# stevenabreu7/SparseRNNs

Measured on AMD Instinct MI355X. Metric: frames/sec at w8a16 S5 dim_scale=0.5 (NDNS shape), bit-exact vs CPU fxprun, higher is better.
Workload: dtype int32

## Files before the change

sparsernns_amd/csrc/proj_p.hpp:

```cpp
#pragma once
#ifdef S5_PHASE_PROF
__device__ long long g_phase_prof[2048 * 8];
#define PHASE_DECL unsigned prof_last, prof_a0 = 0, prof_a1 = 0, prof_a2 = 0, prof_a3 = 0, prof_a4 = 0, prof_a5 = 0, prof_a6 = 0, prof_a7 = 0; \
    { unsigned long long t_; asm volatile("s_memtime %0\n\ts_waitcnt lgkmcnt(0)" : "=s"(t_)); prof_last = __builtin_amdgcn_readfirstlane((unsigned)t_); }
#define PHASE_MARK(i, reg) do { unsigned long long t_; asm volatile("v_cmp_eq_u32 vcc, %1, %1\n\ts_nop 0\n\ts_memtime %0\n\ts_waitcnt lgkmcnt(0)" : "=s"(t_) : "v"(reg) : "memory", "vcc"); \
    const unsigned tl_ = __builtin_amdgcn_readfirstlane((unsigned)t_); prof_a##i = __builtin_amdgcn_readfirstlane(prof_a##i + (tl_ - prof_last)); prof_last = tl_; } while (0)
#define PHASE_DUMP do { if (threadIdx.x == 0 && blockIdx.x < 2048) { long long *o_ = g_phase_prof + blockIdx.x * 8; o_[0] = prof_a0; o_[1] = prof_a1; o_[2] = prof_a2; o_[3] = prof_a3; \
    o_[4] = prof_a4; o_[5] = prof_a5; o_[6] = prof_a6; o_[7] = prof_a7; } } while (0)
#else
#define PHASE_DECL
#define PHASE_MARK(i, reg)
#define PHASE_DUMP
#endif
#include "mfma_bn.hpp"

namespace s5 {

__host__ __device__ constexpr int shape_channels(int NT) { return (NT == 2 || NT == 5) ? 32 * NT - 16 : 32 * NT; }

template <int HC, int HP, int KP>
__device__ __forceinline__ void zero_plane_tail(int8_t *base, int rows)
{
    if constexpr (HC != HP) {
        static_assert(HP - HC == 16, "half a tile");
        for (int i = threadIdx.x; i < rows; i += blockDim.x) *reinterpret_cast<v4i *>(base + i * KP + HC) = v4i{0, 0, 0, 0};
    }
}

__device__ __forceinline__ void planes8_from_i32(const int32_t (&v)[8], v2i &hi, v2i &lo)
{
#pragma unroll
    for (int j = 0; j < 2; ++j) {
        const unsigned p01 = perm((unsigned)v[4 * j + 1], (unsigned)v[4 * j], 0x05010400u);
        const unsigned p23 = perm((unsigned)v[4 * j + 3], (unsigned)v[4 * j + 2], 0x05010400u);
        lo[j] = (int)(perm(p23, p01, 0x05040100u) ^ 0x80808080u);
        hi[j] = (int)perm(p23, p01, 0x07060302u);
    }
}

struct StepRange {
    int32_t t_lo, t_len;
};
template <int FT = 64>
__device__ __forceinline__ void tile_of(int64_t tile, const StepRange &sr, int64_t &b, int &t, int &nvalid)
{
    const int tps = (sr.t_len + FT - 1) / FT;
    b = tile / tps;
    const int tt = (int)(tile - b * tps) * FT;
    t = sr.t_lo + tt;
    nvalid = sr.t_len - tt < FT ? sr.t_len - tt : FT;
}

template <int FT = 64>
struct TileWalk {
    int tps, db, dti;
    int b, ti;
    __device__ __forceinline__ TileWalk(int64_t tile0, const StepRange &sr, unsigned step)
    {
        tps = (sr.t_len + FT - 1) / FT;
        db = (int)(step / (unsigned)tps); dti = (int)(step % (unsigned)tps);
        b = (int)((unsigned)tile0 / (unsigned)tps); ti = (int)((unsigned)tile0 % (unsigned)tps);
    }
    __device__ __forceinline__ void advance()
    {
        b += db; ti += dti;
        if (ti >= tps) { ti -= tps; ++b; }
    }
    __device__ __forceinline__ TileWalk next() const { TileWalk n = *this; n.advance(); return n; }
    __device__ __forceinline__ int t(const StepRange &sr) const { return sr.t_lo + ti * FT; }
    __device__ __forceinline__ int nvalid(const StepRange &sr) const { const int left = sr.t_len - ti * FT; return left < FT ? left : FT; }
};

template <int KS, int NT, bool TRACE, int SM = 0, int NC = NT>
__global__ __launch_bounds__(64 * NT, TRACE ? 2 : KS == 5 ? 3 : 4) void k_bproj_p(BprojM2Args a, GroupOff go)
{
    {
        const int64_t g = blockIdx.y;
        gshift(a.bn.dyn, g * go.ws); gshift(a.bn.xe.dyn, g * go.ws); gshift(a.x, g * go.ws); gshift(a.bq, g * go.ws); gshift(a.u, g * go.ws);
        gshift(a.ext, g * go.ws); gshift(a.status, g * go.status); gshift(a.status_exps, g * go.status);
    }
    static_assert(NC == NT || 2 * NC == NT || 4 * NC == NT, "column tiles per workgroup");
    constexpr int H = shape_channels(KS), HP = 32 * KS, FT = 64, KP = 32 * KS + 16, PC = 16 * NC, SUB0_STEP = NT / NC;
    constexpr int VPF = H / 8;
    constexpr int NTHR = 64 * NT;
    constexpr int NV = FT * VPF / NTHR;
    constexpr int NCT = 1;
    constexpr int PLANE = FT * KP;
    static_assert(FT * VPF % NTHR == 0, "tile shape");
    extern __shared__ __attribute__((aligned(16))) int8_t smem[];
    int32_t *tab = reinterpret_cast<int32_t *>(smem);
    int8_t *Xh = smem + 16 * HP, *Xl = Xh + 2 * PLANE;
    zero_plane_tail<H, HP, KP>(Xh, 4 * FT);
    const int l = threadIdx.x & 63, r = l & 31, h = l >> 5, wave = threadIdx.x >> 6;
    const int wct = wave % NC, wsub = wave / NC;
    const StepRange sr{a.t_lo, a.t_len};
    const int64_t tiles = (a.N / a.L) * ((sr.t_len + FT - 1) / FT);
    int64_t tile = blockIdx.x;

    v4i raw[NV];
    auto fetch = [&](const TileWalk<FT> &tw) {
        const int64_t b = tw.b;
        const int t = tw.t(sr), nv = tw.nvalid(sr);
        const char *xb = reinterpret_cast<const char *>(a.x + (b * a.L + t) * H);
#pragma unroll
        for (int i = 0; i < NV; ++i) {
            const int v = threadIdx.x + NTHR * i;
            int f = v / VPF;
            f = f < nv ? f : nv - 1;
            raw[i] = *reinterpret_cast<const v4i *>(xb + 2u * (unsigned)(f * H + 8 * (v % VPF)));
        }
    };
    TileWalk<FT> walk(tile, sr, gridDim.x);
    if (tile < tiles) fetch(walk);
    v4i wreg[NCT][KS];
    int32_t csv[NCT];
#pragma unroll
    for (int c = 0; c < NCT; ++c) {
        const int col = 32 * (wct + NC * c) + r;
        csv[c] = a.w.cs128[col];
#pragma unroll
        for (int ks = 0; ks < KS; ++ks)
            wreg[c][ks] = *reinterpret_cast<const v4i *>(a.w.wt + (size_t)col * a.w.Kp + 32 * ks + 16 * h);
    }
    const LayerDyn d = a.ext ? bn_finalize_mm_body(a.bn, a.ext, H, const_cast<LayerDyn *>(a.bn.dyn), a.status, a.status_exps, a.bn.xe.get(), a.ext_reps,
                                                   blockIdx.x == 0)
                             : *a.bn.dyn;
    const Bn16 bn = bn16_setup(a.bn, d, tab, H);
    constexpr bool LAZY = KS == 3 && !TRACE;
    ResolveU16 rz{};
    int lazy_arm = 0;
    if constexpr (LAZY) {
        if (a.lazy) {
            gshift_nn(a.lazy, (int64_t)blockIdx.y * go.ws);
            rz = resolve_u16_setup(a.lazy->res.post);
            lazy_arm = 1 + rz.arm;
        }
    }
    __syncthreads();

    prologue_loads_done();
    for (int it = 0; tile < tiles; tile += gridDim.x, ++it, walk.advance()) {
        const int64_t b0 = walk.b;
        const int t0 = walk.t(sr), nvalid = walk.nvalid(sr);
        const int64_t n0 = b0 * a.L + t0;
        char *ub = reinterpret_cast<char *>(a.u + n0 * H);
        int8_t *xh = Xh + (it & 1) * PLANE, *xl = Xl + (it & 1) * PLANE;
#pragma unroll
        for (int i = 0; i < NV; ++i) {
            const int v = threadIdx.x + NTHR * i, f = v / VPF, og = v % VPF;
            const int64_t n = n0 + f;
            int32_t xin[8], t[8], u[8];
            if constexpr (LAZY) {
                if (lazy_arm == 1 + RES_RIGHT) {
#pragma unroll
                    for (int e = 0; e < 4; ++e) raw[i][e] = (int)resolve_u16_pair<RES_RIGHT>(rz, (uint32_t)raw[i][e]);
                } else if (lazy_arm) {
#pragma unroll
                    for (int e = 0; e < 4; ++e) raw[i][e] = (int)resolve_u16_pair<RES_GENERIC>(rz, (uint32_t)raw[i][e]);
                }
            }
            unpack8_i16(raw[i], xin);
            bn16_x4(bn, reinterpret_cast<const int32_t(&)[4]>(xin[0]), 8 * og, reinterpret_cast<int32_t(&)[4]>(t[0]),
                    reinterpret_cast<int32_t(&)[4]>(u[0]));
            bn16_x4(bn, reinterpret_cast<const int32_t(&)[4]>(xin[4]), 8 * og + 4, reinterpret_cast<int32_t(&)[4]>(t[4]),
                    reinterpret_cast<int32_t(&)[4]>(u[4]));
            if (f < nvalid && (TRACE || !a.no_u)) {
                const v2i p0 = pack4_i16(u[0], u[1], u[2], u[3]), p1 = pack4_i16(u[4], u[5], u[6], u[7]);
                *reinterpret_cast<v4i *>(ub + 2u * (unsigned)(f * H + 8 * og)) = v4i{p0[0], p0[1], p1[0], p1[1]};
                if (TRACE) {
#pragma unroll
                    for (int e = 0; e < 8; ++e) {
                        if (a.tr_pre_s5) a.tr_pre_s5[n * H + 8 * og + e] = t[e];
                        if (a.tr_u) a.tr_u[n * H + 8 * og + e] = u[e];
                    }
                }
            }
            v2i hi, lo;
            planes8_from_i32(u, hi, lo);
            *reinterpret_cast<v2i *>(xh + f * KP + 8 * og) = hi;
            *reinterpret_cast<v2i *>(xl + f * KP + 8 * og) = lo;
        }
        if (tile + gridDim.x < tiles) fetch(walk.next());
        __syncthreads();
#pragma unroll
        for (int c = 0; c < NCT; ++c) {
            const int col = 32 * (wct + NC * c) + r;
            const int cc = SM >= 2 ? (r >> 4) : (col >= PC ? 1 : 0), p = SM >= 2 ? 16 * (wct + NC * c) + (r & 15) : col - cc * PC;
            const int rs = cc ? a.rs_im : a.rs_re, bits = cc ? a.bim_bits : a.bre_bits, sh = cc ? a.sh_im : a.sh_re;
            const int lsh = sh < 0 ? -sh : 0, rsh = sh > 0 ? sh : 0;
            SatB sbu;
            sbu.hi = (int32_t)((1u << (bits - 1)) - 1u); sbu.lo = ~sbu.hi;
            asm volatile("" : "+v"(sbu.lo), "+v"(sbu.hi));
#pragma unroll
            for (int sub0 = 0; sub0 < 2; sub0 += SUB0_STEP) {
                const int sub = sub0 + wsub;
                if (SUB0_STEP > 2 && sub >= 2) break;
                const int8_t *rowh = xh + (32 * sub + r) * KP + 16 * h, *rowl = xl + (32 * sub + r) * KP + 16 * h;
                v16i acc;
#pragma unroll
                for (int i = 0; i < 16; ++i) acc[i] = 0;
#pragma unroll
                for (int ks = 0; ks < KS; ++ks)
                    acc = __builtin_amdgcn_mfma_i32_32x32x32_i8(*reinterpret_cast<const v4i *>(rowh + 32 * ks), wreg[c][ks], acc, 0, 0, 0);
#pragma unroll
                for (int i = 0; i < 16; ++i) acc[i] = wadd(wshl(acc[i], 8), csv[c]);
#pragma unroll
                for (int ks = 0; ks < KS; ++ks)
                    acc = __builtin_amdgcn_mfma_i32_32x32x32_i8(*reinterpret_cast<const v4i *>(rowl + 32 * ks), wreg[c][ks], acc, 0, 0, 0);
#pragma unroll
                for (int g = 0; g < 4; ++g) {
                    const int o = 32 * sub + 8 * g + 4 * h;
                    const bool live = o < nvalid;
                    {
                        v4i q;
#pragma unroll
                        for (int e = 0; e < 4; ++e) {
                            const int32_t bu = sat(asr(acc[4 * g + e], rs), sbu);
                            q[e] = asr(wshl(bu, lsh), rsh);
                            if (TRACE && o + e < nvalid) {
                                if (!cc && a.tr_bu_re) a.tr_bu_re[(n0 + o + e) * PC + p] = bu;
                                if (cc && a.tr_bu_im) a.tr_bu_im[(n0 + o + e) * PC + p] = bu;
                            }
                        }
                        if (SM == 3) {
                            const int32_t o0 = __builtin_amdgcn_ds_swizzle(q[0], 0x401f), o2 = __builtin_amdgcn_ds_swizzle(q[2], 0x401f);
                            const v2i item = pack4_i16(o0, o2, q[1], q[3]);
                            if (live && (a.live_slots <= 0 || p < a.live_slots)) {
                                char *qb = reinterpret_cast<char *>(reinterpret_cast<int16_t *>(a.bq) + pair16_half(b0, t0 >> 2, 0, 0, a.TB, PC));
                                const unsigned qo = 2u * (unsigned)((((((p >> 5) * (a.TB >> 1) + (o >> 3)) << 6) + 2 * (p & 31) + cc) * 8) + 4 * ((o >> 2) & 1));
                                *reinterpret_cast<v2i *>(qb + qo) = item;
                            }
                        } else if (SM == 2) {
                            const int32_t kc = cc ? 0 : a.k_re;
                            const int32_t k0 = wadd(wshl(q[0], 16), kc), k2 = wadd(wshl(q[2], 16), kc);
                            v4i item;
                            item[0] = __builtin_amdgcn_ds_swizzle(k0, 0x401f);
                            item[1] = __builtin_amdgcn_ds_swizzle(k2, 0x401f);
                            item[2] = wadd(wshl(q[1], 16), kc);
                            item[3] = wadd(wshl(q[3], 16), kc);
                            if (live) *reinterpret_cast<v4i *>(a.bq + pair_word(b0, (t0 + o) >> 2, p, a.TB, PC) + 4 * cc) = item;
                        } else if (SM == 1) {
                            if (live && (a.live_slots <= 0 || p < a.live_slots))
                                *reinterpret_cast<v2i *>(reinterpret_cast<int16_t *>(a.bq) + native_word(b0, t0 + o, p, cc, a.TB, PC)) =
                                    pack4_i16(q[0], q[1], q[2], q[3]);
                        } else if (live)
                            *reinterpret_cast<v4i *>(a.bq + native_word(b0, t0 + o, p, cc, a.TB, PC)) = q;
                    }
                }
            }
        }
    }
}

using v2u16 = __attribute__((ext_vector_type(2))) unsigned short;

struct CfgOp {
    int l, r, b;
    SatB sb;
    __device__ __forceinline__ int32_t operator()(int32_t d) const { return sat(asr(wshl(d, l), r), sb); }
};
__device__ __forceinline__ CfgOp make_cfg(bool on, int bits, int e, int bits2, int e2)
{
    CfgOp c;
    c.l = on && e2 > e ? e2 - e : 0;
    c.r = on && e > e2 ? e - e2 : 0;
    const int b1 = on && e2 != e ? bits : 32, b2 = on && bits > bits2 ? bits2 : 32;
    c.b = b1 < b2 ? b1 : b2;
    c.sb = sat_bounds(c.b);
    return c;
}

template <int KSTEPS>
__device__ __forceinline__ void mfma_planes(v16i &acc, const v4i (&w)[KSTEPS], const int8_t *rowh, const int8_t *rowl,
                                            const int32_t *cs)
{
#pragma unroll
    for (int i = 0; i < 16; ++i) acc[i] = 0;
#pragma unroll
    for (int ks = 0; ks < KSTEPS; ++ks)
        acc = __builtin_amdgcn_mfma_i32_32x32x32_i8(w[ks], *reinterpret_cast<const v4i *>(rowh + 32 * ks), acc, 0, 0, 0);
#pragma unroll
    for (int g = 0; g < 4; ++g) {
        const v4i c = *reinterpret_cast<const v4i *>(cs + 8 * g);
#pragma unroll
        for (int e = 0; e < 4; ++e) acc[4 * g + e] = wadd(wshl(acc[4 * g + e], 8), c[e]);
    }
#pragma unroll
    for (int ks = 0; ks < KSTEPS; ++ks)
        acc = __builtin_amdgcn_mfma_i32_32x32x32_i8(w[ks], *reinterpret_cast<const v4i *>(rowl + 32 * ks), acc, 0, 0, 0);
}

template <int KSTEPS, int NPL>
__device__ __forceinline__ void mfma_nplanes(v16i &acc, const v4i (&w)[KSTEPS], const int8_t *row0, int plane_stride,
                                             const int32_t *cs)
{
#pragma unroll
    for (int i = 0; i < 16; ++i) acc[i] = 0;
#pragma unroll
    for (int pl = NPL - 1; pl >= 0; --pl) {
        if (pl != NPL - 1) {
#pragma unroll
            for (int g = 0; g < 4; ++g) {
                const v4i c = *reinterpret_cast<const v4i *>(cs + 8 * g);
#pragma unroll
                for (int e = 0; e < 4; ++e) acc[4 * g + e] = wadd(wshl(acc[4 * g + e], 8), c[e]);
            }
        }
#pragma unroll
        for (int ks = 0; ks < KSTEPS; ++ks) {
            acc = __builtin_amdgcn_mfma_i32_32x32x32_i8(w[ks], *reinterpret_cast<const v4i *>(row0 + pl * plane_stride + 32 * ks), acc, 0, 0, 0);
        }
    }
}

enum { IO_I32 = 0, IO_F32 = 1, IO_I16 = 2 };

template <int NT>
__global__ __launch_bounds__(384, 3) void k_enc_p(EncArgs a, float *ext, int ext_reps, GroupOff go)
{
    constexpr int IO = IO_I32;
#include "proj_enc_body.inc"
}

template <int NT>
__global__ __launch_bounds__(384, 3) void k_enc_pf(EncArgs a, float *ext, int ext_reps, GroupOff go)
{
    constexpr int IO = IO_F32;
#include "proj_enc_body.inc"
}

template <int NT>
__global__ __launch_bounds__(384, 3) void k_enc_ps(EncArgs a, float *ext, int ext_reps, GroupOff go)
{
    constexpr int IO = IO_I16;
#include "proj_enc_body.inc"
}

__device__ int32_t g_store_sink[64];
struct DecResid {
    const int16_t *z;
    ResidHead hd;
    int32_t res_bits, skip_bits;
    int32_t usum;
};
template <int KS, bool RESID = false>
__global__ __launch_bounds__(384, KS == 6 && RESID ? 2 : 3) void k_dec_p(DecArgs a, DecResid rz, GroupOff go)
{
    constexpr int IO = IO_I32;
#include "proj_dec_body.inc"
}

template <int KS, bool RESID>
__global__ __launch_bounds__(384, KS == 6 && RESID ? 2 : 3) void k_dec_pf(DecArgs a, DecResid rz, GroupOff go)
{
    constexpr int IO = IO_F32;
#include "proj_dec_body.inc"
}

template <int KS, bool RESID>
__global__ __launch_bounds__(384, KS == 6 ? 2 : 3) void k_dec_ps(DecArgs a, DecResid rz, GroupOff go)
{
    constexpr int IO = IO_I16;
#include "proj_dec_body.inc"
}


}
```

Baseline: 818.2 million.

## Add packed 16-bit row batchnorm fast path for projection phase A

Result: faster. 833.4 million (median of 6 runs) (+1.9%).

```diff
diff --git a/sparsernns_amd/csrc/proj_p.hpp b/sparsernns_amd/csrc/proj_p.hpp
--- a/sparsernns_amd/csrc/proj_p.hpp
+++ b/sparsernns_amd/csrc/proj_p.hpp
@@ -136,6 +136,24 @@
             lazy_arm = 1 + rz.arm;
         }
     }
+    constexpr bool ROW8 = KS == 3 && !TRACE;
+    Bn16Row brow{};
+    int row_arm = ROW_GENERIC;
+    const v4i *rowtab = reinterpret_cast<const v4i *>(tab + 2 * H);
+    if constexpr (ROW8) {
+        if (!a.bn.scale && !a.bn.bias) {
+            bn16_row_shifts(brow, a.bn.xb, a.bn.mb, a.bn.ib, a.bn.b1, a.bn.b2, a.bn.out_bits < a.bn.ub ? a.bn.out_bits : a.bn.ub, d.bn1.shx,
+                            d.bn1.post, d.rs2, a.bn.ue - d.bn_e);
+            row_arm = brow.arm;
+            if (row_arm != ROW_GENERIC && threadIdx.x < H) {
+                const int c = 8 * (threadIdx.x >> 3) + 2 * (threadIdx.x & 3);
+                int32_t p0, p1;
+                if (threadIdx.x & 4) { p0 = a.bn.isv[c]; p1 = a.bn.isv[c + 1]; }
+                else { p0 = sat(wshl(a.bn.mm[c], d.bn1.shy), a.bn.mb); p1 = sat(wshl(a.bn.mm[c + 1], d.bn1.shy), a.bn.mb); }
+                tab[2 * H + threadIdx.x] = (int32_t)(((uint32_t)p0 & 0xffffu) | ((uint32_t)p1 << 16));
+            }
+        }
+    }
     __syncthreads();
 
     prologue_loads_done();
@@ -145,12 +163,13 @@
         const int64_t n0 = b0 * a.L + t0;
         char *ub = reinterpret_cast<char *>(a.u + n0 * H);
         int8_t *xh = Xh + (it & 1) * PLANE, *xl = Xl + (it & 1) * PLANE;
-#pragma unroll
-        for (int i = 0; i < NV; ++i) {
-            const int v = threadIdx.x + NTHR * i, f = v / VPF, og = v % VPF;
-            const int64_t n = n0 + f;
-            int32_t xin[8], t[8], u[8];
-            if constexpr (LAZY) {
+        [[maybe_unused]] auto phase_a_row = [&](auto arm_c) {
+            constexpr int ARM = decltype(arm_c)::value;
+            int tid = threadIdx.x;
+            asm volatile("" : "+v"(tid));
+#pragma unroll
+            for (int i = 0; i < NV; ++i) {
+                const int v = tid + NTHR * i, f = v / VPF, og = v % VPF;
                 if (lazy_arm == 1 + RES_RIGHT) {
 #pragma unroll
                     for (int e = 0; e < 4; ++e) raw[i][e] = (int)resolve_u16_pair<RES_RIGHT>(rz, (uint32_t)raw[i][e]);
@@ -158,27 +177,66 @@
 #pragma unroll
                     for (int e = 0; e < 4; ++e) raw[i][e] = (int)resolve_u16_pair<RES_GENERIC>(rz, (uint32_t)raw[i][e]);
                 }
-            }
-            unpack8_i16(raw[i], xin);
-            bn16_x4(bn, reinterpret_cast<const int32_t(&)[4]>(xin[0]), 8 * og, reinterpret_cast<int32_t(&)[4]>(t[0]),
-                    reinterpret_cast<int32_t(&)[4]>(u[0]));
-            bn16_x4(bn, reinterpret_cast<const int32_t(&)[4]>(xin[4]), 8 * og + 4, reinterpret_cast<int32_t(&)[4]>(t[4]),
-                    reinterpret_cast<int32_t(&)[4]>(u[4]));
-            if (f < nvalid && (TRACE || !a.no_u)) {
-                const v2i p0 = pack4_i16(u[0], u[1], u[2], u[3]), p1 = pack4_i16(u[4], u[5], u[6], u[7]);
-                *reinterpret_cast<v4i *>(ub + 2u * (unsigned)(f * H + 8 * og)) = v4i{p0[0], p0[1], p1[0], p1[1]};
-                if (TRACE) {
-#pragma unroll
-                    for (int e = 0; e < 8; ++e) {
-                        if (a.tr_pre_s5) a.tr_pre_s5[n * H + 8 * og + e] = t[e];
-                        if (a.tr_u) a.tr_u[n * H + 8 * og + e] = u[e];
+                const v4i bm = rowtab[2 * og], bi = rowtab[2 * og + 1];
+                Bn16Row br = brow;
+#pragma unroll
+                for (int k = 0; k < 4; ++k) { br.m[k] = (uint32_t)bm[k]; br.iv[k] = (uint32_t)bi[k]; }
+                const v4i uv = bn16_row8<ARM>(br, raw[i]);
+                if (f < nvalid && !a.no_u) *reinterpret_cast<v4i *>(ub + 2u * (unsigned)(f * H + 8 * og)) = uv;
+                v2i hi, lo;
+#pragma unroll
+                for (int j = 0; j < 2; ++j) {
+                    lo[j] = (int)(perm((unsigned)uv[2 * j + 1], (unsigned)uv[2 * j], 0x06040200u) ^ 0x80808080u);
+                    hi[j] = (int)perm((unsigned)uv[2 * j + 1], (unsigned)uv[2 * j], 0x07050301u);
+                }
+                *reinterpret_cast<v2i *>(xh + f * KP + 8 * og) = hi;
+                *reinterpret_cast<v2i *>(xl + f * KP + 8 * og) = lo;
+            }
+        };
+        bool rows_done = false;
+        if constexpr (ROW8) {
+            if (row_arm != ROW_GENERIC) {
+                if (row_arm == ROW_PACKED) phase_a_row(std::integral_constant<int, ROW_PACKED>{});
+                else phase_a_row(std::integral_constant<int, ROW_SHIFTED>{});
+                rows_done = true;
+            }
+        }
+        if (!rows_done) {
+#pragma unroll
+            for (int i = 0; i < NV; ++i) {
+                const int v = threadIdx.x + NTHR * i, f = v / VPF, og = v % VPF;
+                const int64_t n = n0 + f;
+                int32_t xin[8], t[8], u[8];
+                if constexpr (LAZY) {
+                    if (lazy_arm == 1 + RES_RIGHT) {
+#pragma unroll
+                        for (int e = 0; e < 4; ++e) raw[i][e] = (int)resolve_u16_pair<RES_RIGHT>(rz, (uint32_t)raw[i][e]);
+                    } else if (lazy_arm) {
+#pragma unroll
+                        for (int e = 0; e < 4; ++e) raw[i][e] = (int)resolve_u16_pair<RES_GENERIC>(rz, (uint32_t)raw[i][e]);
                     }
                 }
-            }
-            v2i hi, lo;
-            planes8_from_i32(u, hi, lo);
-            *reinterpret_cast<v2i *>(xh + f * KP + 8 * og) = hi;
-            *reinterpret_cast<v2i *>(xl + f * KP + 8 * og) = lo;
+                unpack8_i16(raw[i], xin);
+                bn16_x4(bn, reinterpret_cast<const int32_t(&)[4]>(xin[0]), 8 * og, reinterpret_cast<int32_t(&)[4]>(t[0]),
+                        reinterpret_cast<int32_t(&)[4]>(u[0]));
+                bn16_x4(bn, reinterpret_cast<const int32_t(&)[4]>(xin[4]), 8 * og + 4, reinterpret_cast<int32_t(&)[4]>(t[4]),
+                        reinterpret_cast<int32_t(&)[4]>(u[4]));
+                if (f < nvalid && (TRACE || !a.no_u)) {
+                    const v2i p0 = pack4_i16(u[0], u[1], u[2], u[3]), p1 = pack4_i16(u[4], u[5], u[6], u[7]);
+                    *reinterpret_cast<v4i *>(ub + 2u * (unsigned)(f * H + 8 * og)) = v4i{p0[0], p0[1], p1[0], p1[1]};
+                    if (TRACE) {
+#pragma unroll
+                        for (int e = 0; e < 8; ++e) {
+                            if (a.tr_pre_s5) a.tr_pre_s5[n * H + 8 * og + e] = t[e];
+                            if (a.tr_u) a.tr_u[n * H + 8 * og + e] = u[e];
+                        }
+                    }
+                }
+                v2i hi, lo;
+                planes8_from_i32(u, hi, lo);
+                *reinterpret_cast<v2i *>(xh + f * KP + 8 * og) = hi;
+                *reinterpret_cast<v2i *>(xl + f * KP + 8 * og) = lo;
+            }
         }
         if (tile + gridDim.x < tiles) fetch(walk.next());
         __syncthreads();
```
